# netidx/netidx

Measured on AMD Instinct MI355X. Metric: Value-batch decode: M updates/s/GPU + GiB/s (device-resident) vs HBM roofline, higher is better.
Workload: dtype u8; 1 GPU; decode 10^7-record all-f64 From::Update batch per GPU (BASELINE configs[1]); records_per_gpu=10000000, wire_bytes_per_gpu=147886336, parallelism=shard-per-gpu x1 (no data-path collective)

## Files before the change

netidx_amd/csrc/nxg_api.cpp:

```cpp
#include <hip/hip_runtime.h>

#include <algorithm>
#include <cstdarg>
#include <cstdio>
#include <cstdlib>
#include <cstring>
#include <mutex>
#include <string>
#include <vector>

#include "../../include/nxg_codec.h"
#include "nxg_internal.h"

namespace {

void set_err(NetidxError* err, const char* fmt, ...) {
    if (!err) return;
    char buf[512];
    va_list ap;
    va_start(ap, fmt);
    vsnprintf(buf, sizeof buf, fmt, ap);
    va_end(ap);
    free(err->msg);
    err->msg = strdup(buf);
}

#define HIPCHK(expr)                                                                       \
    do {                                                                                   \
        hipError_t e_ = (expr);                                                            \
        if (e_ != hipSuccess) {                                                            \
            set_err(err, "%s failed: %s (%s:%d)", #expr, hipGetErrorString(e_), __FILE__,  \
                    __LINE__);                                                             \
            return false;                                                                  \
        }                                                                                  \
    } while (0)

constexpr int kStatusRing = 1024;

}

thread_local uint32_t nxg_patience = 128;
thread_local DevStatus* nxg_zero_slot = nullptr;
thread_local bool nxg_zero_used = false;

struct NxgCtx {
    int device = 0;
    hipStream_t own = nullptr;
    hipStream_t stream = nullptr;
    int ncu = 0;
    int grid_enc_f64 = 0, grid_enc_gen = 0;
    DevStatus* dst = nullptr;
    DevStatus* hst = nullptr;
    uint32_t calls = 0;
    uint32_t epoch = 0;
    uint64_t* tstat = nullptr;
    size_t tstat_words = 0;
    uint32_t* glws = nullptr;
    size_t glws_cap = 0;
    uint64_t* gruns = nullptr;
    bool no_fa = false;
    uint8_t* dscratch = nullptr;
    size_t dscratch_cap = 0;
    int wgs_dec_gen = 0;
    uint8_t* rdesc = nullptr;
    size_t rdesc_cap = 0;
    uint32_t irregular_left = 0;
    bool force_x = false;
    uint32_t seq_left = 0;
    bool no_seq = false;
    uint8_t* pscratch = nullptr;
    size_t pscratch_cap = 0;
    uint32_t enc_seq_left = 0;
    uint32_t last_enc_kernel = 0;
    bool no_enc_seq = false;
    uint32_t mix_left = 0;
    bool no_fmx = false;
    bool fmx_full = false;
    int fmx_count_mode = 0;
    int wgs_fmx[2] = {0, 0};
    uint32_t f64r_flags = 0;
    uint32_t patience = 128;
    uint8_t* dframe = nullptr;
    size_t dframe_cap = 0;
    uint64_t* escratch = nullptr;
    size_t escratch_words = 0;
    NxgColumns dcols{};
    bool dcols_valid = false;
    uint8_t* dheap = nullptr;
    size_t dheap_cap = 0;
    uint8_t* dwflags = nullptr;
    uint64_t* dwid = nullptr;
    size_t dw_cap = 0;
    struct Pending {
        int kind;
        int fast;
        const uint8_t* frame;
        uint64_t len;
        NxgColumns* cols;
        uint64_t* len_out;
        uint64_t cap;
        DevStatus* st;
        uint32_t slot;
        uint32_t flags = 0;
        const uint8_t* heap = nullptr;
        uint8_t* out = nullptr;
    };
    std::vector<Pending> pending;
    void* zdefs = nullptr;
    uint8_t* zlit = nullptr;
    int zgrid = 0;
    void* zrecs = nullptr;
    size_t zrecs_cap = 0;
    void* zc_tables = nullptr;
    uint8_t* zc_slab = nullptr;
    int zc_grid = 0;
    uint8_t* zc_recs = nullptr;
    size_t zc_recs_cap = 0;
    uint8_t* zc_out = nullptr;
    size_t zc_out_cap = 0;
    uint8_t* zc_pack = nullptr;
    size_t zc_pack_cap = 0;
    uint8_t* zc_hpin = nullptr;
    size_t zc_hpin_cap = 0;
    hipEvent_t zc_ev[2] = {nullptr, nullptr};
    float zc_kernel_ms = 0.f;
    DevStatus last{};
    uint64_t fa_last[8] = {};
    uint8_t* aw_dev = nullptr;
    size_t aw_dev_cap = 0;
    uint8_t* aw_host = nullptr;
    size_t aw_host_cap = 0;
    uint64_t last_split = 0;
};

namespace {

bool set_device(NxgCtx* c, NetidxError* err) {
    HIPCHK(hipSetDevice(c->device));
    return true;
}

bool begin_call(NxgCtx* c, DevStatus** st, uint32_t* slot, NetidxError* err) {
    *slot = c->calls % kStatusRing;
    *st = c->dst + *slot;
    nxg_patience = c->patience;
    nxg_zero_slot = c->dst + (c->calls + kStatusRing / 2) % kStatusRing;
    nxg_zero_used = false;
    c->calls++;
    c->epoch++;
    if (c->epoch > kEpochMax) {
        c->epoch = 1;
        if (c->tstat) HIPCHK(hipMemsetAsync(c->tstat, 0, c->tstat_words * 8, c->stream));
    }
    return true;
}

bool end_call(NxgCtx* c, NetidxError* err) {
    if (nxg_zero_used) return true;
    nxg_zero_used = true;
    HIPCHK(hipMemsetAsync(nxg_zero_slot, 0, sizeof(DevStatus), c->stream));
    return true;
}

bool ensure_tstat(NxgCtx* c, size_t words, NetidxError* err) {
    if (words <= c->tstat_words) return true;
    size_t n = std::max(words, c->tstat_words * 2);
    n = std::max<size_t>(n, 4096);
    HIPCHK(hipStreamSynchronize(c->stream));
    if (c->tstat) HIPCHK(hipFree(c->tstat));
    c->tstat = nullptr;
    HIPCHK(hipMalloc(&c->tstat, n * 8));
    HIPCHK(hipMemsetAsync(c->tstat, 0, n * 8, c->stream));
    c->tstat_words = n;
    return true;
}

bool ensure_escratch(NxgCtx* c, size_t words, NetidxError* err) {
    if (words <= c->escratch_words) return true;
    HIPCHK(hipStreamSynchronize(c->stream));
    if (c->escratch) HIPCHK(hipFree(c->escratch));
    c->escratch = nullptr;
    size_t n = std::max<size_t>(words, 1024);
    HIPCHK(hipMalloc(&c->escratch, n * 8));
    c->escratch_words = n;
    return true;
}

bool is_device_ptr(const void* p) {
    if (!p) return false;
    hipPointerAttribute_t a;
    if (hipPointerGetAttributes(&a, p) != hipSuccess) {
        (void)hipGetLastError();
        return false;
    }
    return a.type == hipMemoryTypeDevice;
}
// ... 526 lines not shown
    c->device = device;
    auto fail = [&](const char* what, hipError_t e) -> NxgCtx* {
        set_err(err, "%s: %s", what, hipGetErrorString(e));
        delete c;
        return nullptr;
    };
    hipError_t e;
    if ((e = hipSetDevice(device)) != hipSuccess) return fail("hipSetDevice", e);
    hipDeviceProp_t prop;
    if ((e = hipGetDeviceProperties(&prop, device)) != hipSuccess)
        return fail("hipGetDeviceProperties", e);
    if (strncmp(prop.gcnArchName, "gfx950", 6) != 0) {
        set_err(err, "nxg codec is built for gfx950 (MI355X); device %d is %s", device,
                prop.gcnArchName);
        delete c;
        return nullptr;
    }
    c->ncu = prop.multiProcessorCount;
    if ((e = hipStreamCreateWithFlags(&c->own, hipStreamNonBlocking)) != hipSuccess)
        return fail("hipStreamCreate", e);
    c->stream = c->own;
    auto grid = [&](int occ) { return c->ncu * std::max(1, occ > 2 ? occ - 1 : occ); };
    const char* pe = getenv("NXG_PERSISTENT");
    const bool persist = pe && pe[0] == '1';
    c->grid_enc_f64 = persist ? grid(nxg_occupancy_enc_f64()) : 0;
    c->grid_enc_gen = persist ? grid(nxg_occupancy_enc_general()) : 0;
    if ((e = hipMalloc(&c->dst, sizeof(DevStatus) * kStatusRing)) != hipSuccess)
        return fail("hipMalloc(status)", e);
    if ((e = hipMemset(c->dst, 0, sizeof(DevStatus) * kStatusRing)) != hipSuccess)
        return fail("hipMemset(status)", e);
    if ((e = hipHostMalloc(&c->hst, sizeof(DevStatus) * (kStatusRing + 1), hipHostMallocDefault)) !=
        hipSuccess)
        return fail("hipHostMalloc(status)", e);
    const size_t gw = (size_t)gdec2::MAX_RUNS * (gdec2::RUN_WORDS + 4);
    if ((e = hipMalloc(&c->gruns, gw * 8)) != hipSuccess) return fail("hipMalloc(gruns)", e);
    c->wgs_dec_gen = nxg_dec_gen_wgs(c->ncu);
    nxg_fmx_wgs(c->ncu, c->wgs_fmx);
    const char* fp = getenv("NXG_F64_PATH");
    c->force_x = fp && strcmp(fp, "x") == 0;
    c->no_seq = fp && (strcmp(fp, "run") == 0 || strcmp(fp, "x") == 0);
    const char* fe = getenv("NXG_F64_ENC");
    c->no_enc_seq = fe && strcmp(fe, "tile") == 0;
    const char* mp = getenv("NXG_MIXED_PATH");
    c->no_fmx = mp && strcmp(mp, "general") == 0;
    const char* fc = getenv("NXG_FMX_COUNT");
    c->fmx_count_mode = fc && strcmp(fc, "full") == 0 ? 1 : (fc && strcmp(fc, "lean") == 0 ? 2 : 0);
    const char* ap = getenv("NXG_ARCH_PATH");
    c->no_fa = ap && strcmp(ap, "exact") == 0;
    const char* lp = getenv("NXG_LOOKBACK_PATIENCE");
    c->patience = lp ? (uint32_t)strtoul(lp, nullptr, 0) : 128u;
    const char* ff = getenv("NXG_F64R_FLAGS");
    c->f64r_flags = ff ? (uint32_t)strtoul(ff, nullptr, 0) : 0u;
    return c;
}

void nxg_ctx_destroy(NxgCtx* c) {
    if (!c) return;
    (void)hipSetDevice(c->device);
    if (c->stream) (void)hipStreamSynchronize(c->stream);
    if (c->dcols_valid) cols_free_impl(&c->dcols);
    if (c->tstat) (void)hipFree(c->tstat);
    if (c->glws) (void)hipFree(c->glws);
    if (c->gruns) (void)hipFree(c->gruns);
    if (c->dscratch) (void)hipFree(c->dscratch);
    if (c->pscratch) (void)hipFree(c->pscratch);
    if (c->dframe) (void)hipFree(c->dframe);
// ... 103 lines not shown
        target->n_children = s.n_children;
        target->n_ctl = s.n_ctl;
        if (s.err_kind == 0) {
            NxgColumns hv = *out;
            if (s.path == 1) hv.tag = nullptr;
            if (!copy_cols_d2h(c, target, &hv, err)) return false;
        }
    }
    out->n_rows = s.n_rows;
    out->n_children = s.n_children;
    out->n_ctl = s.n_ctl;
    out->n_heartbeat = s.n_heartbeat;
    if (ust) *ust = s;
    return true;
}

bool nxg_decode_updates_async(NxgCtx* c, const uint8_t* dframe, uint64_t len, NxgColumns* dout,
                              uint32_t flags, NetidxError* err) {
    if (!c || !dout || (!dframe && len)) {
        set_err(err, "null argument");
        return false;
    }
    if (c->pending.size() >= kStatusRing / 2) {
        set_err(err, "too many in-flight async calls (max %d); call nxg_ctx_sync", kStatusRing / 2);
        return false;
    }
    if (dout->mem != NXG_MEM_DEVICE || ((uintptr_t)dframe & 15)) {
        set_err(err, "async decode needs device columns and a 16-byte aligned device frame");
        return false;
    }
    DevStatus* st;
    uint32_t slot;
    if (!begin_call(c, &st, &slot, err)) return false;
    int fast = FAST_NONE;
    const bool ok = !(flags & NXG_DECODE_HINT_MIXED)
                        ? enqueue_dec_fast(c, dframe, len, dout, st, &fast, err)
                        : enqueue_dec_mixed(c, dframe, len, dout, st, &fast, err);
    if (!end_call(c, err) || !ok) return false;
    c->pending.push_back({1, fast, dframe, len, dout, nullptr, 0, st, slot, flags});
    return true;
}

bool nxg_decode_frames_async(NxgCtx* c, uint32_t n, const uint8_t* const* dframes,
                             const uint64_t* lens, NxgColumns* const* douts, uint32_t flags,
                             NetidxError* err) {
    if (!c || (n && (!dframes || !lens || !douts))) {
        set_err(err, "null argument");
        return false;
    }
    if (c->pending.size() + n > kStatusRing / 2) {
        set_err(err, "too many in-flight async calls (max %d); call nxg_ctx_sync", kStatusRing / 2);
        return false;
    }
    uint64_t max_len = 0;
    for (uint32_t j = 0; j < n; j++) {
        if (!douts[j] || (!dframes[j] && lens[j])) {
            set_err(err, "null frame or columns at %u", j);
            return false;
        }
        if (douts[j]->mem != NXG_MEM_DEVICE || ((uintptr_t)dframes[j] & 15)) {
            set_err(err, "async decode needs device columns and 16-byte aligned device frames");
            return false;
        }
        max_len = std::max(max_len, lens[j]);
    }
    const bool run_path = !(flags & NXG_DECODE_HINT_MIXED) && !c->force_x &&
                          c->irregular_left == 0 && n > 1 && !seq_active(c);
    if (!run_path) {
        for (uint32_t j = 0; j < n; j++)
            if (!nxg_decode_updates_async(c, dframes[j], lens[j], douts[j], flags, err))
                return false;
        return true;
    }
    if (!set_device(c, err)) return false;
    const size_t half = (16 * nxg_dec_f64r_tiles(max_len) + 255) & ~(size_t)255;
    if (!ensure_tstat(c, nxg_dec_f64r_groups(max_len), err)) return false;
    if (!ensure_rdesc(c, 2 * half, err)) return false;
    std::vector<NxgF64rFrame> fr(n);
    std::vector<NxgCtx::Pending> pend;
    pend.reserve(n);
    uint32_t nonempty = 0;
    for (uint32_t j = 0; j < n; j++) {
        DevStatus* st;
        uint32_t slot;
        if (!begin_call(c, &st, &slot, err)) return false;
        NxgF64rFrame& f = fr[j];
        f.wire = dframes[j];
        f.W = lens[j];
        f.oid = douts[j]->id;
        f.oval = douts[j]->fixed;
        f.cap = douts[j]->cap_rows;
        f.desc = c->rdesc + (nonempty & 1) * half;
        if (lens[j]) nonempty++;
        f.epoch = c->epoch;
        f.st = st;
        f.zst = nxg_take_zero_slot();
        if (lens[j] == 0) HIPCHK(hipMemsetAsync(f.zst, 0, sizeof(DevStatus), c->stream));
        pend.push_back({1, FAST_RUN, dframes[j], lens[j], douts[j], nullptr, 0, st, slot});
    }
    HIPCHK(nxg_launch_dec_f64r_stream(fr.data(), n, c->tstat, c->f64r_flags, c->stream));
    c->seq_left = c->seq_left > n ? c->seq_left - n : 0;
    c->pending.insert(c->pending.end(), pend.begin(), pend.end());
    return true;
}

bool nxg_ctx_sync(NxgCtx* c, NxgStatus* ust, NetidxError* err) {
    if (!c) {
        set_err(err, "null ctx");
        return false;
    }
    if (!set_device(c, err)) return false;
    std::vector<NxgCtx::Pending> ps;
    ps.swap(c->pending);
    HIPCHK(hipStreamSynchronize(c->stream));
    std::vector<DevStatus> hs(ps.size());
    if (!ps.empty()) {
        const uint32_t s0 = ps.front().slot, s1 = ps.back().slot;
        if (s0 <= s1) {
            HIPCHK(hipMemcpyAsync(c->hst + s0, c->dst + s0, sizeof(DevStatus) * (s1 - s0 + 1),
                                  hipMemcpyDeviceToHost, c->stream));
        } else {
            HIPCHK(hipMemcpyAsync(c->hst + s0, c->dst + s0, sizeof(DevStatus) * (kStatusRing - s0),
                                  hipMemcpyDeviceToHost, c->stream));
            HIPCHK(hipMemcpyAsync(c->hst, c->dst, sizeof(DevStatus) * (s1 + 1),
                                  hipMemcpyDeviceToHost, c->stream));
        }
        HIPCHK(hipStreamSynchronize(c->stream));
        for (size_t i = 0; i < ps.size(); i++) hs[i] = c->hst[ps[i].slot];
    }
    if (ust) memset(ust, 0, sizeof *ust);
    bool reported = false, ok = true;
    std::vector<Span> dirty;
    auto written_later = [&](size_t i, const std::vector<Span>& rd) {
        for (size_t j = i + 1; j < ps.size(); j++) {
            std::vector<Span> wj;
            if (ps[j].kind == 1) cols_spans(ps[j].cols, &wj);
            else wj.push_back(span_of(ps[j].out, ps[j].cap));
            if (overlaps(rd, wj)) return true;
        }
        return false;
    };
    for (size_t i = 0; i < ps.size(); i++) {
        auto& p = ps[i];
        c->hst[p.slot] = hs[i];
        NetidxError e{nullptr};
        bool r;
        if (p.kind == 1) {
            std::vector<Span> w;
            cols_spans(p.cols, &w);
            const std::vector<Span> fr = {span_of(p.frame, p.len)};
            const bool stale = !dirty.empty() && (overlaps(dirty, w) || overlaps(dirty, fr));
            const bool reread = stale || (hs[i].fast_fail && p.fast);
            NxgStatus s;
            bool redone = false;
            if (reread && p.len > 0 && !covered(dirty, fr) && written_later(i, fr)) {
                if (ok) {
                    ok = false;
                    set_err(err, "decode of async call %zu needs its frame again (%s), "
                                 "but a later call in the backlog wrote into that frame "
                                 "buffer; keep a frame unchanged until nxg_ctx_sync",
                            i, stale ? "redone after an earlier call's fallback" : "fallback");
                }
                continue;
            }
            if (stale) {
                r = redo_decode(c, p, &s, &e);
                redone = true;
            } else {
                r = finish_decode(c, p.frame, p.len, p.cols, p.fast, p.st, p.slot, &s, &e, true,
                                  &redone);
            }
            if (redone) dirty.insert(dirty.end(), w.begin(), w.end());
            if (r) {
                p.cols->layout =
                    (!mixed_capable(p.cols) || s.path == 1) ? NXG_LAYOUT_F64 : NXG_LAYOUT_MIXED;
                if (ust && !reported) *ust = s;
                if (s.err_kind) reported = true;
            }
        } else {
            NxgColumns dummy{};
            dummy.layout = NXG_LAYOUT_F64;
            const NxgColumns* in = p.cols ? p.cols : &dummy;
            std::vector<Span> rd;
            cols_spans(in, &rd);
            const Span wr = span_of(p.out, p.cap);
            const bool stale = !dirty.empty() && (overlaps(dirty, rd) || overlaps(dirty, {wr}));
            const bool reread = stale || (p.fast && hs[i].fast_fail);
            if (reread && !covered(dirty, rd) && written_later(i, rd)) {
                r = false;
                set_err(&e, "encode of async call %zu needs its columns again (%s), but a "
                            "later call in the backlog wrote into them; keep them unchanged until "
                            "nxg_ctx_sync", i,
                        stale ? "redone after an earlier call's fallback" : "fallback");
            } else if (stale) {
                r = redo_encode(c, p, in, &e);
                dirty.push_back(wr);
            } else {
                bool redone = false;
                r = finish_encode(c, in, p.st, p.slot, p.len_out, p.cap, true, &e, true, p.fast,
                                  p.heap, p.out, &redone);
                if (redone) dirty.push_back(wr);
            }
        }
        if (!r && ok) {
            ok = false;
// ... 1333 lines not shown
}

bool nxg_encoded_writes_len(NxgCtx* c, const NxgColumns* in, const NxgWriteCols* win,
                            const uint8_t* heap, uint64_t* len_out, NetidxError* err) {
    if (!writes_args_ok(c, in, win, err)) return false;
    return encode_impl(c, in, heap, nullptr, 0, len_out, err, win);
}

bool nxg_encode_writes(NxgCtx* c, const NxgColumns* in, const NxgWriteCols* win,
                       const uint8_t* heap, uint8_t* out, uint64_t cap, uint64_t* len_out,
                       NetidxError* err) {
    if (!writes_args_ok(c, in, win, err)) return false;
    return encode_impl(c, in, heap, out, cap, len_out, err, win);
}

bool nxg_encode_updates_async(NxgCtx* c, const NxgColumns* din, const uint8_t* dheap,
                              uint8_t* dout, uint64_t cap, uint64_t* len_out, NetidxError* err) {
    if (!c || !din || !dout) {
        set_err(err, "null argument");
        return false;
    }
    if (c->pending.size() >= kStatusRing / 2) {
        set_err(err, "too many in-flight async calls (max %d); call nxg_ctx_sync", kStatusRing / 2);
        return false;
    }
    for (auto& p : c->pending)
        if (p.kind == 2 && din->layout == NXG_LAYOUT_MIXED && din->n_ctl) {
            set_err(err, "sync the previous encode before an async encode with control spans");
            return false;
        }
    DevStatus* st;
    uint32_t slot;
    if (!begin_call(c, &st, &slot, err)) return false;
    int fast = 0;
    const bool ok = enqueue_encode(c, din, dheap, dout, cap, st, err, &fast);
    if (!end_call(c, err) || !ok) return false;
    c->pending.push_back({2, fast, nullptr, 0, const_cast<NxgColumns*>(din), len_out, cap, st,
                          slot, 0, dheap, dout});
    return true;
}

bool nxg_encode_frames(NxgCtx* c, const NxgColumns* in, const uint8_t* heap, uint8_t* out,
                       uint64_t cap, uint64_t* len_out, uint64_t* chunk_len_out,
                       uint64_t cap_chunks, uint64_t* n_chunks, NetidxError* err) {
    if (!out || !n_chunks || (cap_chunks && !chunk_len_out)) {
        set_err(err, "null argument");
        return false;
    }
    uint64_t total = 0;
    if (!encode_impl(c, in, heap, out, cap, &total, err)) return false;
    if (len_out) *len_out = total;
    uint64_t ch[2];
    uint64_t k = 0;
    if (total == 0) {
        k = 0;
    } else if (total <= kMaxBatch) {
        ch[k++] = total;
    } else {
        if (!c->last_split) {
            set_err(err, "frame split: the encoder recorded no boundary for a %llu-byte batch",
                    (unsigned long long)total);
            return false;
        }
        const uint64_t c1 = c->last_split - 1;
        if (total > kMaxBatch + c1) {
            set_err(err, "frame split: a %llu-byte batch needs more than one cut (the reference "
                         "then cuts before every message); split the batch or use "
                         "nxg_frame_split with the message lengths", (unsigned long long)total);
            return false;
        }
        ch[k++] = c1;
// ... 401 lines not shown
```

netidx_amd/csrc/nxg_decode_f64_seq.hip:

```cpp
#include "nxg_device.h"
#include "nxg_f64_rec16.h"

namespace f64s {
constexpr int TPB = 256;
#ifndef NXG_F64S_R
#define NXG_F64S_R 8
#endif
#ifndef NXG_F64S_R_SMALL
#define NXG_F64S_R_SMALL 4
#endif
#ifndef NXG_F64S_NT
#define NXG_F64S_NT 1
#endif
constexpr uint64_t kXcdMin = 256ull << 20;
inline int r_for(uint64_t W) { return W >= kXcdMin ? NXG_F64S_R : NXG_F64S_R_SMALL; }
#ifndef NXG_F64S_XCD
#define NXG_F64S_XCD 1
#endif
#ifndef NXG_F64S_LDS
#define NXG_F64S_LDS 0
#endif
constexpr uint32_t F_XCD = 1;
#ifndef NXG_F64S_XRUN
#define NXG_F64S_XRUN 64
// ... 77 lines not shown
        d[7] = wave_next(A[r].w);
        uint4 nx;
        if (r + 1 < R) {
            nx = make_uint4((uint32_t)__builtin_amdgcn_readfirstlane((int)A[r + 1].x),
                            (uint32_t)__builtin_amdgcn_readfirstlane((int)A[r + 1].y),
                            (uint32_t)__builtin_amdgcn_readfirstlane((int)A[r + 1].z),
                            (uint32_t)__builtin_amdgcn_readfirstlane((int)A[r + 1].w));
        } else {
            nx = E;
        }
        if (lane == 63) {
            d[4] = nx.x, d[5] = nx.y, d[6] = nx.z, d[7] = nx.w;
        }
        const uint32_t k = r * 64 + lane;
        const uint32_t Lk = k < ks ? L : L2;
        uint32_t e0, e1, e2, e3;
        extract16(d, o[r] & 15u, e0, e1, e2, e3);
        uint64_t id, val;
        rec_decode16(e0, e1, e2, e3, Lk, id, val);
        bad |= (rec_check16(e0, e1, W - (a0 + o[r])) != Lk) | (id != ib + k);
        const uint64_t row = k0 + k;
        if (row < cap) {
            st_col(&oid[row], id);
            st_col(&oval[row], val);
        } else {
            over = true;
        }
    }
    return bad;
}

#ifndef NXG_F64S_PAIR
#define NXG_F64S_PAIR 1
#endif
template <int R>
NXG_DEV bool emit_full_pairs(const uint8_t* __restrict__ wire, uint64_t W, uint64_t p0, uint32_t L,
                             uint32_t ks, uint64_t k0, uint64_t i0, uint64_t* __restrict__ oid,
                             uint64_t* __restrict__ oval, uint64_t cap, uint32_t lane,
                             bool& over) {
    using namespace f64rec16;
    constexpr int RP = R / 2;
    const uint64_t a0 = p0 & ~15ull;
    const uint8_t* __restrict__ base = wire + a0;
    const uint32_t s0 = (uint32_t)(p0 & 15u);
    const uint32_t L2 = L + 1;
    auto off = [&](uint32_t k) -> uint32_t {
        return s0 + (k < ks ? k * L : ks * L + (k - ks) * L2);
    };
    uint4 A[RP], B[RP], Cq[RP];
    uint32_t oa[RP], ob[RP];
#pragma unroll
    for (int r = 0; r < RP; r++) {
        const uint32_t k = 2 * (r * 64 + lane);
        oa[r] = off(k);
        ob[r] = off(k + 1);
        const uint32_t ab = oa[r] & ~15u;
        A[r] = ld16s(base + ab);
        B[r] = ld16s(base + ab + 16);
        if (lane == 63) Cq[r] = ld16s(base + ab + 32);
    }
    bool bad = false;
    const uint64_t ib = i0 + k0;
#pragma unroll
    for (int r = 0; r < RP; r++) {
        const uint32_t k = 2 * (r * 64 + lane);
        const uint32_t ab = oa[r] & ~15u;
// ... 20 lines not shown
        const uint32_t d2[8] = {up ? B[r].x : A[r].x, up ? B[r].y : A[r].y, up ? B[r].z : A[r].z,
                                up ? B[r].w : A[r].w, up ? C[0] : B[r].x, up ? C[1] : B[r].y,
                                up ? C[2] : B[r].z, up ? C[3] : B[r].w};
        extract16(d2, sb & 15u, e0, e1, e2, e3);
        uint64_t idb, vb;
        rec_decode16(e0, e1, e2, e3, Lb, idb, vb);
        bad |= (rec_check16(e0, e1, W - (a0 + ob[r])) != Lb) | (idb != ib + k + 1);
        const uint64_t row = k0 + k;
        if (row + 1 < cap) {
            const uint4 iv = make_uint4((uint32_t)ida, (uint32_t)(ida >> 32), (uint32_t)idb,
                                        (uint32_t)(idb >> 32));
            const uint4 vv = make_uint4((uint32_t)va, (uint32_t)(va >> 32), (uint32_t)vb,
                                        (uint32_t)(vb >> 32));
            if (NXG_F64S_NT & 1) {
                __builtin_nontemporal_store(*reinterpret_cast<const v4u*>(&iv),
                                            reinterpret_cast<v4u*>(oid + row));
                __builtin_nontemporal_store(*reinterpret_cast<const v4u*>(&vv),
                                            reinterpret_cast<v4u*>(oval + row));
            } else {
                *reinterpret_cast<uint4*>(oid + row) = iv;
                *reinterpret_cast<uint4*>(oval + row) = vv;
            }
        } else {
            if (row < cap) {
                oid[row] = ida;
                oval[row] = va;
            }
            over = true;
        }
    }
    return bad;
}

}

template <int R>
__global__ __launch_bounds__(f64s::TPB) void nxg_f64s_kernel(const uint8_t* __restrict__ wire,
                                                             uint64_t W, uint64_t* __restrict__ oid,
                                                             uint64_t* __restrict__ oval,
                                                             uint64_t cap, uint32_t flags,
                                                             DevStatus* __restrict__ st,
                                                             DevStatus* zst) {
    using namespace f64s;
    using namespace f64rec16;
    constexpr uint32_t WREC = 64 * R;
    const uint32_t failed = st->fast_fail;
    zero_status(zst);
    const uint32_t lane = threadIdx.x & 63;
    const uint32_t w = (uint32_t)__builtin_amdgcn_readfirstlane((int)(threadIdx.x >> 6));
    uint4 h0;
    if (W >= 16) {
        h0 = *reinterpret_cast<const uint4*>(wire);
    } else {
        uint32_t v[4] = {0, 0, 0, 0};
        for (uint32_t k = 0; k < (uint32_t)W; k++) v[k >> 2] |= (uint32_t)wire[k] << (8 * (k & 3));
        h0 = make_uint4(v[0], v[1], v[2], v[3]);
    }
    h0.x = (uint32_t)__builtin_amdgcn_readfirstlane((int)h0.x);
    h0.y = (uint32_t)__builtin_amdgcn_readfirstlane((int)h0.y);
    h0.z = (uint32_t)__builtin_amdgcn_readfirstlane((int)h0.z);
    h0.w = (uint32_t)__builtin_amdgcn_readfirstlane((int)h0.w);
    const uint32_t hl = rec_check16(h0.x, h0.y, W);
    if (!hl) {
        if (blockIdx.x == 0 && threadIdx.x == 0) {
            atomicOr(&st->irregular, 2u);
            atomicOr(&st->fast_fail, 1u);
        }
        return;
    }
    uint64_t i0, v0;
    rec_decode16(h0.x, h0.y, h0.z, h0.w, hl, i0, v0);
    uint64_t blk = blockIdx.x;
    if (flags & F_XCD) {
        const uint64_t full = (uint64_t)gridDim.x / (8 * XRUN) * (8 * XRUN);
        if (blk < full) {
            const uint64_t x = blk % 8, k = blk / 8;
            blk = ((k / XRUN) * 8 + x) * XRUN + k % XRUN;
        }
    }
    const uint64_t k0 = (blk * (TPB / 64) + w) * WREC;
    const uint64_t p0 = pos_of(i0, k0);
    if (p0 >= W || failed) return;
    const uint64_t id0 = i0 + k0;
    const uint32_t b = vl64(id0);
    const uint64_t nxt = 1ull << (7 * b);
    const uint32_t L = 11u + b;
    const uint32_t ks = nxt - id0 < WREC ? (uint32_t)(nxt - id0) : WREC;
    const uint64_t pend = p0 + (uint64_t)ks * L + (uint64_t)(WREC - ks) * (L + 1);
    bool over = false, bad = b > 5;
    if (!bad && pend + 48 <= W) {
        bad = NXG_F64S_PAIR ? emit_full_pairs<R>(wire, W, p0, L, ks, k0, i0, oid, oval, cap, lane, over)
                            : emit_full<R>(wire, W, p0, L, ks, k0, i0, oid, oval, cap, lane, over);
    } else if (!bad) {
        uint32_t n = WREC;
        if (pend > W) {
            uint32_t lo = 0, hi = WREC;
            while (hi - lo > 1) {
                const uint32_t mid = (lo + hi) / 2;
                if (pos_of(i0, k0 + mid) < W) lo = mid;
                else hi = mid;
            }
            n = hi;
        }
        const uint64_t pn = pos_of(i0, k0 + n);
        if (pn == W && lane == 0) {
            st->n_rows = k0 + n;
            st->path = 1;
            st->diag[1] = 1;
        }
        if (pn < W && n < WREC) bad = true;
        else if (pn > W) bad = true;
        else bad = emit_edge(wire, W, p0, L, ks, n, k0, i0, oid, oval, cap, lane, over);
    }
    if (__any(bad) && lane == 0) {
        atomicOr(&st->irregular, 4u);
        atomicOr(&st->fast_fail, 1u);
    }
    if (__any(over) && lane == 0) atomicOr(&st->capacity, 1u);
}

uint64_t nxg_dec_f64s_groups(uint64_t W) {
    const uint64_t maxrec = W / 12 + 1;
    const uint64_t wrec = 64ull * (uint64_t)f64s::r_for(W);
    const uint64_t waves = (maxrec + wrec - 1) / wrec;
    return (waves + f64s::TPB / 64 - 1) / (f64s::TPB / 64);
// ... 17 lines not shown
```

netidx_amd/csrc/nxg_f64_rec16.h:

```cpp
#pragma once
#include "nxg_device.h"

namespace f64rec16 {

NXG_DEV uint64_t seq_pos(uint64_t i0, uint64_t k) {
    uint64_t p = 12 * k;
#pragma unroll
    for (uint32_t t = 1; t <= 4; t++) {
        const uint64_t B = 1ull << (7 * t);
        const uint64_t x = i0 + k > B ? i0 + k - B : 0ull;
        p += x < k ? x : k;
    }
    return p;
}

NXG_DEV uint4 ld16r(const uint8_t* __restrict__ p) { return *reinterpret_cast<const uint4*>(p); }
__device__ __attribute__((noinline)) uint4 ld16_tail(const uint8_t* __restrict__ wire,
                                                    uint64_t off, uint64_t W) {
    uint32_t v[4] = {0, 0, 0, 0};
#pragma unroll
    for (int k = 0; k < 16; k++)
        if (off + k < W) v[k >> 2] |= (uint32_t)wire[off + k] << (8 * (k & 3));
    return make_uint4(v[0], v[1], v[2], v[3]);
}
// ... 10 lines not shown
#pragma unroll
    for (int j = 0; j < 6; j++) g[j] = d[j] ^ ((d[j] ^ d[j + 2]) & m2);
#pragma unroll
    for (int j = 0; j < 5; j++) f[j] = g[j] ^ ((g[j] ^ g[j + 1]) & m1);
    e0 = alignbyte(f[1], f[0], r);
    e1 = alignbyte(f[2], f[1], r);
    e2 = alignbyte(f[3], f[2], r);
    e3 = alignbyte(f[4], f[3], r);
}

NXG_DEV uint32_t rec_check16(uint32_t e0, uint32_t e1, uint64_t rem) {
    const uint32_t L = e0 & 0xffu;
    const bool head = (L - 12u <= 4u) && (((e0 >> 8) & 0xffu) == 4u);
    const uint32_t sh = 8u * ((L - 11u) & 7u);
    const uint64_t x = ((((uint64_t)e1) << 32) | e0) >> 16;
    const uint64_t m = (1ull << sh) - 1ull;
    const uint64_t want = 0x8080808080ull & (m >> 8);
    const bool var = (x & 0x808080808080ull & m) == want;
    const uint32_t tag = (uint32_t)(x >> sh) & 0xffu;
    return (head && var && tag == 9u && rem >= L) ? L : 0u;
}

NXG_DEV void rec_decode16(uint32_t e0, uint32_t e1, uint32_t e2, uint32_t e3, uint32_t L,
                          uint64_t& id, uint64_t& val) {
    const uint32_t sh = 8u * ((L - 11u) & 7u);
    const uint64_t x = ((((uint64_t)e1) << 32) | e0) >> 16;
    const uint64_t y = x & ((1ull << sh) - 1ull) & 0x7f7f7f7f7full;
    id = (y & 0x7full) | ((y >> 1) & 0x3f80ull) | ((y >> 2) & 0x1fc000ull) |
         ((y >> 3) & 0xfe00000ull) | ((y >> 4) & 0x7f0000000ull);
    const uint32_t o = L - 8u;
    const uint32_t lo = o >= 8u ? e2 : alignbyte(e2, e1, o & 3u);
    const uint32_t hi = o >= 8u ? e3 : alignbyte(e3, e2, o & 3u);
    val = ((uint64_t)bswap32(lo) << 32) | bswap32(hi);
}

NXG_DEV uint32_t len_bytes(uint32_t x) {
    const uint32_t y = x & 0x7f7f7f7fu;
    return (0x90909090u - y) & ~x & (y + 0x74747474u) & 0x80808080u;
}
NXG_DEV uint32_t cand16(uint32_t d0, uint32_t d1, uint32_t d2, uint32_t d3, uint32_t d4) {
    const uint32_t a = nib(len_bytes(d0)) | (nib(len_bytes(d1)) << 4) | (nib(len_bytes(d2)) << 8) |
                       (nib(len_bytes(d3)) << 12);
    const uint32_t b = nib(zero_bytes(d0 ^ 0x04040404u)) | (nib(zero_bytes(d1 ^ 0x04040404u)) << 4) |
                       (nib(zero_bytes(d2 ^ 0x04040404u)) << 8) |
                       (nib(zero_bytes(d3 ^ 0x04040404u)) << 12) |
                       (nib(zero_bytes(d4 ^ 0x04040404u)) << 16);
    return a & (b >> 1) & 0xffffu;
}

struct LinImg {
    const uint8_t* b;
    NXG_DEV uint32_t w(uint32_t i) const { return reinterpret_cast<const uint32_t*>(b)[i]; }
    NXG_DEV uint32_t byte(uint32_t p) const { return b[p]; }
};
struct SwzImg {
    const uint8_t* b;
    static NXG_DEV uint32_t sw(uint32_t i) { return i ^ ((i >> 4) & 15u); }
    NXG_DEV uint32_t w(uint32_t i) const { return reinterpret_cast<const uint32_t*>(b)[sw(i)]; }
    NXG_DEV uint32_t byte(uint32_t p) const { return b[(sw(p >> 2) << 2) | (p & 3u)]; }
};

template <typename Img>
NXG_DEV void lds16i(const Img& im, uint32_t rel, uint32_t& e0, uint32_t& e1, uint32_t& e2,
                   uint32_t& e3) {
    const uint32_t q = rel >> 2, s = rel & 3u;
    const uint32_t d0 = im.w(q), d1 = im.w(q + 1), d2 = im.w(q + 2), d3 = im.w(q + 3),
// ... 182 lines not shown
```

netidx_amd/csrc/nxg_internal.h:

```cpp
#pragma once
#include <hip/hip_runtime.h>
#include <stdint.h>

#include "../../include/nxg_codec.h"

struct DevStatus {
    uint64_t n_rows, n_children, n_ctl, n_heartbeat;
    uint32_t err_kind;
    uint32_t path;
    uint64_t err_offset;
    uint32_t fast_fail;
    uint32_t timeout;
    uint32_t capacity;
    uint32_t runs_valid;
    uint64_t total_bytes;
    uint32_t nonf64;
    uint32_t irregular;
    uint64_t err_key;
    uint64_t split_start;
    unsigned long long diag[8];
};
static_assert(sizeof(DevStatus) == 160, "DevStatus layout");

constexpr uint64_t kFlagAgg = 1ull << 62;
// ... 14 lines not shown
__host__ __device__ inline uint64_t lb_flag(uint64_t w, uint32_t epoch) {
    return ((w >> kEpochShift) & kEpochMax) == epoch ? (w & kFlagMask) : 0ull;
}

namespace gdec2 {
constexpr int TPB = 256;
constexpr int CH = 64;
constexpr uint32_t TILE = 64 * CH;
constexpr uint32_t IMG = TILE + 1024;
constexpr int MAX_RUNS = 8192;
constexpr int RUN_WORDS = 8;
}

namespace f64enc {
constexpr int LB_U = 1;
constexpr int TPB = 256;
constexpr int RPT = 4;
constexpr int TILE = TPB * RPT;
constexpr int MAXB = TILE * 15 + 32;
}

extern thread_local uint32_t nxg_patience;

struct ColsDesc;
__device__ inline void zero_status(DevStatus* zst) {
    if (zst && blockIdx.x == 0 && threadIdx.x == 0) *zst = DevStatus{};
}
extern thread_local DevStatus* nxg_zero_slot;
extern thread_local bool nxg_zero_used;
inline DevStatus* nxg_take_zero_slot() {
    nxg_zero_used = true;
    return nxg_zero_slot;
}
uint64_t nxg_dec_f64x_groups(uint64_t W);
hipError_t nxg_launch_dec_f64x_range(const uint8_t* wire, uint64_t W, uint64_t begin,
                                     uint64_t end, uint64_t* oid, uint64_t* oval, uint64_t cap,
                                     uint64_t* tstat, uint32_t epoch, DevStatus* st,
                                     hipStream_t s);
hipError_t nxg_launch_dec_f64x(const uint8_t* wire, uint64_t W, uint64_t* oid, uint64_t* oval,
                               uint64_t cap, uint64_t* tstat, uint32_t epoch, DevStatus* st,
                               hipStream_t s);
uint64_t nxg_dec_f64s_groups(uint64_t W);
hipError_t nxg_launch_dec_f64s(const uint8_t* wire, uint64_t W, uint64_t* oid, uint64_t* oval,
                               uint64_t cap, DevStatus* st, DevStatus* zst, hipStream_t s);
uint64_t nxg_dec_f64r_tiles(uint64_t W);
uint64_t nxg_dec_f64r_tile_bytes();
uint64_t nxg_dec_f64r_groups(uint64_t W);
hipError_t nxg_launch_dec_f64r(const uint8_t* wire, uint64_t W, uint64_t begin, uint64_t end,
                               uint64_t* oid, uint64_t* oval, uint64_t cap, void* desc,
                               uint64_t* tstat, uint32_t epoch, uint32_t flags, DevStatus* st,
                               hipStream_t s);
struct NxgF64rFrame {
    const uint8_t* wire;
    uint64_t W;
    uint64_t* oid;
    uint64_t* oval;
    uint64_t cap;
    void* desc;
    uint32_t epoch;
    DevStatus* st;
    DevStatus* zst;
};
hipError_t nxg_launch_dec_f64r_stream(const NxgF64rFrame* fr, uint32_t n, uint64_t* tstat,
                                      uint32_t flags, hipStream_t s);
uint64_t nxg_enc_f64_tiles(uint64_t n);
hipError_t nxg_launch_enc_f64(const uint64_t* id, const uint64_t* val, uint64_t n, uint8_t* out,
// ... 166 lines not shown
```

Before: 182,800 M updates/s.

## Gather status via mapped-host kernel and add uniform-length f64 seq decode path

Replaces the per-sync device-to-host memcpy of status slots with a small kernel that writes the status ring directly into mapped pinned host memory, enqueued at the end of each batched decode. This removes the extra copy, synchronization and round trip at sync time. It also adds a specialised pair-emission path for the f64 sequential decoder when all records in a wave share the same length, which uses cheaper header checks and value extraction. Finally, sync skips computing span lists when nothing is dirty. The risks are more code paths to keep correct and an extra kernel launch per batch.

```diff
diff --git a/netidx_amd/csrc/nxg_api.cpp b/netidx_amd/csrc/nxg_api.cpp
--- a/netidx_amd/csrc/nxg_api.cpp
+++ b/netidx_amd/csrc/nxg_api.cpp
@@ -51,7 +51,9 @@
     int grid_enc_f64 = 0, grid_enc_gen = 0;
     DevStatus* dst = nullptr;
     DevStatus* hst = nullptr;
+    DevStatus* hst_dev = nullptr;
     uint32_t calls = 0;
+    uint32_t gathered_to = 0;
     uint32_t epoch = 0;
     uint64_t* tstat = nullptr;
     size_t tstat_words = 0;
@@ -104,6 +106,7 @@
         uint32_t flags = 0;
         const uint8_t* heap = nullptr;
         uint8_t* out = nullptr;
+        uint32_t seq = 0;
     };
     std::vector<Pending> pending;
     void* zdefs = nullptr;
@@ -162,6 +165,24 @@
     return true;
 }
 
+bool gather_pending(NxgCtx* c, NetidxError* err) {
+    if (c->pending.empty()) return true;
+    const uint32_t first = c->pending.front().seq;
+    const uint32_t span = c->pending.back().seq - first + 1;
+    uint32_t done = c->gathered_to - first;
+    if (done > span) done = 0;
+    if (done == span) return true;
+    HIPCHK(nxg_launch_status_gather(c->dst, c->hst_dev, (first + done) % kStatusRing,
+                                    std::min<uint32_t>(span - done, kStatusRing), kStatusRing,
+                                    c->stream));
+    c->gathered_to = first + span;
+    return true;
+}
+
+void gather_forget(NxgCtx* c) {
+    c->gathered_to = c->pending.empty() ? c->calls : c->pending.front().seq;
+}
+
 bool ensure_tstat(NxgCtx* c, size_t words, NetidxError* err) {
     if (words <= c->tstat_words) return true;
     size_t n = std::max(words, c->tstat_words * 2);
@@ -754,6 +775,8 @@
     if ((e = hipHostMalloc(&c->hst, sizeof(DevStatus) * (kStatusRing + 1), hipHostMallocDefault)) !=
         hipSuccess)
         return fail("hipHostMalloc(status)", e);
+    if ((e = hipHostGetDevicePointer((void**)&c->hst_dev, c->hst, 0)) != hipSuccess)
+        return fail("hipHostGetDevicePointer(status)", e);
     const size_t gw = (size_t)gdec2::MAX_RUNS * (gdec2::RUN_WORDS + 4);
     if ((e = hipMalloc(&c->gruns, gw * 8)) != hipSuccess) return fail("hipMalloc(gruns)", e);
     c->wgs_dec_gen = nxg_dec_gen_wgs(c->ncu);
@@ -923,22 +946,24 @@
     DevStatus* st;
     uint32_t slot;
     if (!begin_call(c, &st, &slot, err)) return false;
+    const uint32_t seq = c->calls - 1;
     int fast = FAST_NONE;
     const bool ok = !(flags & NXG_DECODE_HINT_MIXED)
                         ? enqueue_dec_fast(c, dframe, len, dout, st, &fast, err)
                         : enqueue_dec_mixed(c, dframe, len, dout, st, &fast, err);
     if (!end_call(c, err) || !ok) return false;
     c->pending.push_back({1, fast, dframe, len, dout, nullptr, 0, st, slot, flags});
-    return true;
-}
-
-bool nxg_decode_frames_async(NxgCtx* c, uint32_t n, const uint8_t* const* dframes,
-                             const uint64_t* lens, NxgColumns* const* douts, uint32_t flags,
-                             NetidxError* err) {
-    if (!c || (n && (!dframes || !lens || !douts))) {
-        set_err(err, "null argument");
-        return false;
-    }
+    c->pending.back().seq = seq;
+    return true;
+}
+
+}
+
+namespace {
+
+bool decode_frames_async_impl(NxgCtx* c, uint32_t n, const uint8_t* const* dframes,
+                              const uint64_t* lens, NxgColumns* const* douts, uint32_t flags,
+                              NetidxError* err) {
     if (c->pending.size() + n > kStatusRing / 2) {
         set_err(err, "too many in-flight async calls (max %d); call nxg_ctx_sync", kStatusRing / 2);
         return false;
@@ -961,7 +986,7 @@
         for (uint32_t j = 0; j < n; j++)
             if (!nxg_decode_updates_async(c, dframes[j], lens[j], douts[j], flags, err))
                 return false;
-        return true;
+        return gather_pending(c, err);
     }
     if (!set_device(c, err)) return false;
     const size_t half = (16 * nxg_dec_f64r_tiles(max_len) + 255) & ~(size_t)255;
@@ -988,11 +1013,28 @@
         f.zst = nxg_take_zero_slot();
         if (lens[j] == 0) HIPCHK(hipMemsetAsync(f.zst, 0, sizeof(DevStatus), c->stream));
         pend.push_back({1, FAST_RUN, dframes[j], lens[j], douts[j], nullptr, 0, st, slot});
+        pend.back().seq = c->calls - 1;
     }
     HIPCHK(nxg_launch_dec_f64r_stream(fr.data(), n, c->tstat, c->f64r_flags, c->stream));
     c->seq_left = c->seq_left > n ? c->seq_left - n : 0;
     c->pending.insert(c->pending.end(), pend.begin(), pend.end());
-    return true;
+    return gather_pending(c, err);
+}
+
+}
+
+extern "C" {
+
+bool nxg_decode_frames_async(NxgCtx* c, uint32_t n, const uint8_t* const* dframes,
+                             const uint64_t* lens, NxgColumns* const* douts, uint32_t flags,
+                             NetidxError* err) {
+    if (!c || (n && (!dframes || !lens || !douts))) {
+        set_err(err, "null argument");
+        return false;
+    }
+    if (decode_frames_async_impl(c, n, dframes, lens, douts, flags, err)) return true;
+    gather_forget(c);
+    return false;
 }
 
 bool nxg_ctx_sync(NxgCtx* c, NxgStatus* ust, NetidxError* err) {
@@ -1001,24 +1043,18 @@
         return false;
     }
     if (!set_device(c, err)) return false;
+    const bool gathered = gather_pending(c, err);
     std::vector<NxgCtx::Pending> ps;
     ps.swap(c->pending);
+    if (!gathered) {
+        (void)hipStreamSynchronize(c->stream);
+        c->gathered_to = c->calls;
+        return false;
+    }
     HIPCHK(hipStreamSynchronize(c->stream));
+    c->gathered_to = c->calls;
     std::vector<DevStatus> hs(ps.size());
-    if (!ps.empty()) {
-        const uint32_t s0 = ps.front().slot, s1 = ps.back().slot;
-        if (s0 <= s1) {
-            HIPCHK(hipMemcpyAsync(c->hst + s0, c->dst + s0, sizeof(DevStatus) * (s1 - s0 + 1),
-                                  hipMemcpyDeviceToHost, c->stream));
-        } else {
-            HIPCHK(hipMemcpyAsync(c->hst + s0, c->dst + s0, sizeof(DevStatus) * (kStatusRing - s0),
-                                  hipMemcpyDeviceToHost, c->stream));
-            HIPCHK(hipMemcpyAsync(c->hst, c->dst, sizeof(DevStatus) * (s1 + 1),
-                                  hipMemcpyDeviceToHost, c->stream));
-        }
-        HIPCHK(hipStreamSynchronize(c->stream));
-        for (size_t i = 0; i < ps.size(); i++) hs[i] = c->hst[ps[i].slot];
-    }
+    for (size_t i = 0; i < ps.size(); i++) hs[i] = c->hst[ps[i].slot];
     if (ust) memset(ust, 0, sizeof *ust);
     bool reported = false, ok = true;
     std::vector<Span> dirty;
@@ -1037,13 +1073,16 @@
         NetidxError e{nullptr};
         bool r;
         if (p.kind == 1) {
-            std::vector<Span> w;
-            cols_spans(p.cols, &w);
-            const std::vector<Span> fr = {span_of(p.frame, p.len)};
+            NxgStatus s;
+            bool redone = false;
+            const bool plain = dirty.empty() && !hs[i].fast_fail;
+            std::vector<Span> w, fr;
+            if (!plain) {
+                cols_spans(p.cols, &w);
+                fr.push_back(span_of(p.frame, p.len));
+            }
             const bool stale = !dirty.empty() && (overlaps(dirty, w) || overlaps(dirty, fr));
             const bool reread = stale || (hs[i].fast_fail && p.fast);
-            NxgStatus s;
-            bool redone = false;
             if (reread && p.len > 0 && !covered(dirty, fr) && written_later(i, fr)) {
                 if (ok) {
                     ok = false;
@@ -1061,7 +1100,10 @@
                 r = finish_decode(c, p.frame, p.len, p.cols, p.fast, p.st, p.slot, &s, &e, true,
                                   &redone);
             }
-            if (redone) dirty.insert(dirty.end(), w.begin(), w.end());
+            if (redone) {
+                if (plain) cols_spans(p.cols, &w);
+                dirty.insert(dirty.end(), w.begin(), w.end());
+            }
             if (r) {
                 p.cols->layout =
                     (!mixed_capable(p.cols) || s.path == 1) ? NXG_LAYOUT_F64 : NXG_LAYOUT_MIXED;
@@ -2461,11 +2503,12 @@
     DevStatus* st;
     uint32_t slot;
     if (!begin_call(c, &st, &slot, err)) return false;
+    const uint32_t seq = c->calls - 1;
     int fast = 0;
     const bool ok = enqueue_encode(c, din, dheap, dout, cap, st, err, &fast);
     if (!end_call(c, err) || !ok) return false;
     c->pending.push_back({2, fast, nullptr, 0, const_cast<NxgColumns*>(din), len_out, cap, st,
-                          slot, 0, dheap, dout});
+                          slot, 0, dheap, dout, seq});
     return true;
 }
 
diff --git a/netidx_amd/csrc/nxg_decode_f64_seq.hip b/netidx_amd/csrc/nxg_decode_f64_seq.hip
--- a/netidx_amd/csrc/nxg_decode_f64_seq.hip
+++ b/netidx_amd/csrc/nxg_decode_f64_seq.hip
@@ -133,6 +133,9 @@
 
 #ifndef NXG_F64S_PAIR
 #define NXG_F64S_PAIR 1
+#endif
+#ifndef NXG_F64S_UNIFORM
+#define NXG_F64S_UNIFORM 1
 #endif
 template <int R>
 NXG_DEV bool emit_full_pairs(const uint8_t* __restrict__ wire, uint64_t W, uint64_t p0, uint32_t L,
@@ -219,6 +222,91 @@
     return bad;
 }
 
+template <int R>
+NXG_DEV bool emit_full_pairs_uniform(const uint8_t* __restrict__ wire, uint64_t p0, uint32_t L,
+                                     uint64_t k0, uint64_t i0, uint64_t* __restrict__ oid,
+                                     uint64_t* __restrict__ oval, uint64_t cap, uint32_t lane,
+                                     bool& over) {
+    using namespace f64rec16;
+    constexpr int RP = R / 2;
+    const uint64_t a0 = p0 & ~15ull;
+    const uint8_t* __restrict__ base = wire + a0;
+    const uint32_t s0 = (uint32_t)(p0 & 15u);
+    const uint32_t nb = L - 11u;
+    const uint64_t hc = seq_head_const(nb), hm = seq_head_mask(nb);
+    const uint32_t c0 = (uint32_t)hc, c1 = (uint32_t)(hc >> 32);
+    const uint32_t m0 = (uint32_t)hm, m1 = (uint32_t)(hm >> 32);
+    uint4 A[RP], B[RP], Cq[RP];
+    uint32_t oa[RP];
+#pragma unroll
+    for (int r = 0; r < RP; r++) {
+        const uint32_t k = 2 * (r * 64 + lane);
+        oa[r] = s0 + k * L;
+        const uint32_t ab = oa[r] & ~15u;
+        A[r] = ld16s(base + ab);
+        B[r] = ld16s(base + ab + 16);
+        if (lane == 63) Cq[r] = ld16s(base + ab + 32);
+    }
+    uint32_t bad = 0;
+    const uint64_t ib = i0 + k0;
+#pragma unroll
+    for (int r = 0; r < RP; r++) {
+        const uint32_t k = 2 * (r * 64 + lane);
+        const uint32_t ab = oa[r] & ~15u;
+        const uint32_t nA[4] = {wave_next(A[r].x), wave_next(A[r].y), wave_next(A[r].z),
+                                wave_next(A[r].w)};
+        const uint32_t nB[4] = {wave_next(B[r].x), wave_next(B[r].y), wave_next(B[r].z),
+                                wave_next(B[r].w)};
+        const bool at32 = ((oa[r] + 2 * L) & ~15u) == ab + 32;
+        uint32_t C[4];
+        C[0] = at32 ? nA[0] : nB[0];
+        C[1] = at32 ? nA[1] : nB[1];
+        C[2] = at32 ? nA[2] : nB[2];
+        C[3] = at32 ? nA[3] : nB[3];
+        if (lane == 63) C[0] = Cq[r].x, C[1] = Cq[r].y, C[2] = Cq[r].z, C[3] = Cq[r].w;
+        const uint64_t ida = ib + k, idb = ida + 1;
+        uint32_t h0, h1;
+        const uint32_t d[8] = {A[r].x, A[r].y, A[r].z, A[r].w, B[r].x, B[r].y, B[r].z, B[r].w};
+        uint32_t e0, e1, e2, e3;
+        extract16(d, oa[r] & 15u, e0, e1, e2, e3);
+        seq_head_id(ida, h0, h1);
+        bad |= ((e0 ^ (h0 | c0)) & m0) | ((e1 ^ (h1 | c1)) & m1);
+        const uint64_t va = rec_value16(e1, e2, e3, L);
+        const uint32_t sb = (oa[r] & 15u) + L;
+        const bool up = sb >= 16;
+        const uint32_t d2[8] = {up ? B[r].x : A[r].x, up ? B[r].y : A[r].y, up ? B[r].z : A[r].z,
+                                up ? B[r].w : A[r].w, up ? C[0] : B[r].x, up ? C[1] : B[r].y,
+                                up ? C[2] : B[r].z, up ? C[3] : B[r].w};
+        extract16(d2, sb & 15u, e0, e1, e2, e3);
+        seq_head_id(idb, h0, h1);
+        bad |= ((e0 ^ (h0 | c0)) & m0) | ((e1 ^ (h1 | c1)) & m1);
+        const uint64_t vb = rec_value16(e1, e2, e3, L);
+        const uint64_t row = k0 + k;
+        if (row + 1 < cap) {
+            const uint4 iv = make_uint4((uint32_t)ida, (uint32_t)(ida >> 32), (uint32_t)idb,
+                                        (uint32_t)(idb >> 32));
+            const uint4 vv = make_uint4((uint32_t)va, (uint32_t)(va >> 32), (uint32_t)vb,
+                                        (uint32_t)(vb >> 32));
+            if (NXG_F64S_NT & 1) {
+                __builtin_nontemporal_store(*reinterpret_cast<const v4u*>(&iv),
+                                            reinterpret_cast<v4u*>(oid + row));
+                __builtin_nontemporal_store(*reinterpret_cast<const v4u*>(&vv),
+                                            reinterpret_cast<v4u*>(oval + row));
+            } else {
+                *reinterpret_cast<uint4*>(oid + row) = iv;
+                *reinterpret_cast<uint4*>(oval + row) = vv;
+            }
+        } else {
+            if (row < cap) {
+                oid[row] = ida;
+                oval[row] = va;
+            }
+            over = true;
+        }
+    }
+    return bad != 0;
+}
+
 }
 
 template <int R>
@@ -276,8 +364,12 @@
     const uint64_t pend = p0 + (uint64_t)ks * L + (uint64_t)(WREC - ks) * (L + 1);
     bool over = false, bad = b > 5;
     if (!bad && pend + 48 <= W) {
-        bad = NXG_F64S_PAIR ? emit_full_pairs<R>(wire, W, p0, L, ks, k0, i0, oid, oval, cap, lane, over)
-                            : emit_full<R>(wire, W, p0, L, ks, k0, i0, oid, oval, cap, lane, over);
+        if (NXG_F64S_PAIR && NXG_F64S_UNIFORM && ks == WREC)
+            bad = emit_full_pairs_uniform<R>(wire, p0, L, k0, i0, oid, oval, cap, lane, over);
+        else
+            bad = NXG_F64S_PAIR
+                      ? emit_full_pairs<R>(wire, W, p0, L, ks, k0, i0, oid, oval, cap, lane, over)
+                      : emit_full<R>(wire, W, p0, L, ks, k0, i0, oid, oval, cap, lane, over);
     } else if (!bad) {
         uint32_t n = WREC;
         if (pend > W) {
diff --git a/netidx_amd/csrc/nxg_f64_rec16.h b/netidx_amd/csrc/nxg_f64_rec16.h
--- a/netidx_amd/csrc/nxg_f64_rec16.h
+++ b/netidx_amd/csrc/nxg_f64_rec16.h
@@ -66,6 +66,26 @@
     const uint32_t lo = o >= 8u ? e2 : alignbyte(e2, e1, o & 3u);
     const uint32_t hi = o >= 8u ? e3 : alignbyte(e3, e2, o & 3u);
     val = ((uint64_t)bswap32(lo) << 32) | bswap32(hi);
+}
+
+NXG_DEV uint64_t seq_head_const(uint32_t nb) {
+    const uint64_t cont = 0x8080808080ull & ((1ull << (8u * (nb - 1u))) - 1ull);
+    return (uint64_t)(11u + nb) | (4ull << 8) | (cont << 16) | (9ull << (8u * (2u + nb)));
+}
+NXG_DEV uint64_t seq_head_mask(uint32_t nb) { return ~0ull >> (8u * (5u - nb)); }
+NXG_DEV void seq_head_id(uint64_t id, uint32_t& h0, uint32_t& h1) {
+    const uint32_t lo = (uint32_t)id, hi = (uint32_t)(id >> 32);
+    const uint32_t v = (lo & 0x7fu) | ((lo << 1) & 0x7f00u) | ((lo << 2) & 0x7f0000u) |
+                       ((lo << 3) & 0x7f000000u);
+    const uint32_t g4 = (lo >> 28) | ((hi & 7u) << 4);
+    h0 = v << 16;
+    h1 = (v >> 16) | (g4 << 16);
+}
+NXG_DEV uint64_t rec_value16(uint32_t e1, uint32_t e2, uint32_t e3, uint32_t L) {
+    const uint32_t o = L - 8u;
+    const uint32_t lo = o >= 8u ? e2 : alignbyte(e2, e1, o & 3u);
+    const uint32_t hi = o >= 8u ? e3 : alignbyte(e3, e2, o & 3u);
+    return ((uint64_t)bswap32(lo) << 32) | bswap32(hi);
 }
 
 NXG_DEV uint32_t len_bytes(uint32_t x) {
diff --git a/netidx_amd/csrc/nxg_internal.h b/netidx_amd/csrc/nxg_internal.h
--- a/netidx_amd/csrc/nxg_internal.h
+++ b/netidx_amd/csrc/nxg_internal.h
@@ -70,6 +70,8 @@
     nxg_zero_used = true;
     return nxg_zero_slot;
 }
+hipError_t nxg_launch_status_gather(const DevStatus* dst, DevStatus* hst_dev, uint32_t s0,
+                                    uint32_t n, uint32_t ring, hipStream_t s);
 uint64_t nxg_dec_f64x_groups(uint64_t W);
 hipError_t nxg_launch_dec_f64x_range(const uint8_t* wire, uint64_t W, uint64_t begin,
                                      uint64_t end, uint64_t* oid, uint64_t* oval, uint64_t cap,
diff --git a/netidx_amd/csrc/nxg_status.hip b/netidx_amd/csrc/nxg_status.hip
--- /dev/null
+++ b/netidx_amd/csrc/nxg_status.hip
@@ -0,0 +1,33 @@
+#include "nxg_device.h"
+#include "nxg_internal.h"
+
+namespace {
+
+constexpr int TPB = 256;
+constexpr uint32_t Q = sizeof(DevStatus) / 16;
+static_assert(sizeof(DevStatus) % 16 == 0, "DevStatus is copied in 16-byte words");
+
+__global__ __launch_bounds__(TPB) void nxg_status_gather_kernel(const DevStatus* __restrict__ dst,
+                                                                DevStatus* __restrict__ hst,
+                                                                uint32_t s0, uint32_t n,
+                                                                uint32_t ring) {
+    const uint4* __restrict__ src = reinterpret_cast<const uint4*>(dst);
+    uint4* __restrict__ out = reinterpret_cast<uint4*>(hst);
+#pragma unroll 1
+    for (uint32_t i = threadIdx.x; i < n * Q; i += TPB) {
+        const uint32_t slot = (s0 + i / Q) % ring;
+        const uint32_t w = slot * Q + i % Q;
+        out[w] = src[w];
+    }
+}
+
+}
+
+hipError_t nxg_launch_status_gather(const DevStatus* dst, DevStatus* hst_dev, uint32_t s0,
+                                    uint32_t n, uint32_t ring, hipStream_t s) {
+    if (n == 0) return hipSuccess;
+    if (n > ring || s0 >= ring) return hipErrorInvalidValue;
+    hipLaunchKernelGGL(nxg_status_gather_kernel, dim3(1), dim3(TPB), 0, s, dst, hst_dev, s0, n,
+                       ring);
+    return hipGetLastError();
+}
```

Result: faster. 185,700 M updates/s, median of 6 (+1.6%).
